# widkyyu/Goal-conditioned-Reinforcement-Learning-with-environmental-and-policy-priors

Measured on AMD Instinct MI355X. Metric: env-steps/sec, higher is better.
Workload: dtype u8

## Files before the change

### goal-conditioned-reinforcement-learning-with-environmental-and-policy-priors_amd/csrc/twoarmy_engine.hip

```cpp

#include <hip/hip_runtime.h>
#include <stdint.h>
#include <stdio.h>
#include <stdlib.h>
#include <string.h>

#include <array>
#include <map>
#include <mutex>
#include <type_traits>
#include <utility>
#include <vector>

#include "launch.h"
#include "philox.h"
#include "twoarmy.h"

namespace {

constexpr int GS = TW_GRID;
constexpr int NC = TW_CELLS;
constexpr int REC = TW_REC_WORDS;

constexpr uint32_t C_EMPTY = 1u;
constexpr uint32_t C_WALL = 2u | (5u << 8);
constexpr uint32_t C_BALL = 6u | (4u << 8);
constexpr uint32_t C_GOAL = 8u | (1u << 8);

constexpr uint32_t M_FREE = 0x3f666666u;
constexpr uint32_t M_WALL = 0xbf666666u;
constexpr uint32_t M_BALL = 0xbf000000u;
constexpr uint32_t M_AGENT = 0x3e99999au;

constexpr int GPW = 33, GPX0 = 8, GPY0 = 16, GPP = 35;
constexpr int GP_WORDS = GPW * GPP;
constexpr int MAT_OFF = 1156;
constexpr int MAT_WORDS = 292;
constexpr int MATC_OFF = MAT_OFF + MAT_WORDS;
constexpr int MATC_BYTES = 304;
constexpr int ENV_WORDS = MATC_OFF + MATC_BYTES / 4;
constexpr int STAGE_WORDS = 220;
constexpr int REC_OBS_OFF = MAT_WORDS * 4;
static_assert(REC_OBS_OFF + 880 == 2048, "matrix row + view-17 image row are exactly 2048 bytes");

enum { R_STEP = 0, R_RISK = 1, R_HIT = 2, R_ROOM2 = 3, R_GOAL = 4 };

struct Params {
    uint8_t *type;
    uint8_t *colour;
    int32_t *rec;
    uint8_t *type_out;
    uint8_t *colour_out;
    int32_t *rec_out;
    int *abnormal;
    int *abnormal_other;
    int only_if_flagged;
    int *fb_count;
    int n_envs;
    int view;
    int variant;
    uint32_t seed_lo, seed_hi;
    uint32_t env_id0;
    int T;
    const int32_t *actions;
    const uint32_t *draws;
    uint8_t *obs;
    float *matrix;
    float *pos;
    float *reward;
    uint8_t *term;
    uint8_t *trunc;
    int obs_pitch;
    int mat_pitch;
    int flags;
    int record;
    const uint32_t *pipe_tab;
};

__device__ __forceinline__ void draw_block(uint32_t k0, uint32_t k1, uint32_t env_id, uint32_t t, uint32_t block,
                                           uint32_t (&w)[4]) {
    w[0] = env_id; w[1] = t; w[2] = block; w[3] = 0x54574F41u;
    philox4x32_10(k0, k1, w[0], w[1], w[2], w[3]);
}

__device__ __forceinline__ uint32_t gen_cell(int x, int y) {
    if (x == 0 || y == 0 || x == GS - 1 || y == GS - 1) return C_WALL;
    if (y == 8) {
        if (x <= 5 || x >= 11) return C_WALL;
        if (x >= 7 && x <= 9) return C_BALL;
        return C_EMPTY;
    }
    if (x == 14 && y == 2) return C_GOAL;
    return C_EMPTY;
}

__device__ __forceinline__ uint32_t mat_of_code(uint32_t code) {
    const uint32_t t = code & 0xffu;
    return t == 2u ? M_WALL : (t == 6u ? M_BALL : M_FREE);
}

struct EnvS {
    int ax, ay, dir, step_count, step_move, m6, m4, pone, patrol, up1, right2, upd_long, upd_horiz, risk,
        first_room2;
    int obx[3], oby[3], o1x[3], o1y[3], o1v, o2x[4], o2y[4], o2v, gx, gy;
    uint32_t t;
    int err, max_steps, episodes, last_reward, last_term, last_trunc;
    int wall_i1, wall_i2;
};

__device__ __forceinline__ void load_env(EnvS &s, const int32_t *r) {
    s.ax = r[TW_AX]; s.ay = r[TW_AY]; s.dir = r[TW_DIR];
    s.step_count = r[TW_STEP_COUNT]; s.step_move = r[TW_STEP_MOVE];
    s.m6 = (int)((uint32_t)s.step_move % 6u); s.m4 = s.step_move & 3;
    s.pone = r[TW_PONE]; s.patrol = r[TW_PATROL]; s.up1 = r[TW_UP1];
    s.right2 = r[TW_RIGHT2]; s.upd_long = r[TW_UPD_LONG]; s.upd_horiz = r[TW_UPD_HORIZ];
    s.risk = r[TW_RISK]; s.first_room2 = r[TW_FIRST_ROOM2];
#pragma unroll
    for (int k = 0; k < 3; ++k) {
        s.obx[k] = r[TW_OBX + k]; s.oby[k] = r[TW_OBY + k];
        s.o1x[k] = r[TW_O1X + k]; s.o1y[k] = r[TW_O1Y + k];
    }
#pragma unroll
    for (int k = 0; k < 4; ++k) { s.o2x[k] = r[TW_O2X + k]; s.o2y[k] = r[TW_O2Y + k]; }
    s.o1v = r[TW_O1_VALID]; s.o2v = r[TW_O2_VALID];
    s.gx = r[TW_GOAL_X]; s.gy = r[TW_GOAL_Y];
    s.t = (uint32_t)r[TW_T]; s.err = r[TW_ERROR]; s.max_steps = r[TW_MAX_STEPS];
    s.episodes = r[TW_EPISODES]; s.last_reward = r[TW_LAST_REWARD];
    s.last_term = r[TW_LAST_TERM]; s.last_trunc = r[TW_LAST_TRUNC];
    s.wall_i1 = r[TW_WALL_I1]; s.wall_i2 = r[TW_WALL_I2];
}

__device__ __forceinline__ void store_env(const EnvS &s, int32_t *r) {
    r[TW_AX] = s.ax; r[TW_AY] = s.ay; r[TW_DIR] = s.dir;
    r[TW_STEP_COUNT] = s.step_count; r[TW_STEP_MOVE] = s.step_move;
    r[TW_PONE] = s.pone; r[TW_PATROL] = s.patrol; r[TW_UP1] = s.up1; r[TW_RIGHT2] = s.right2;
    r[TW_UPD_LONG] = s.upd_long; r[TW_UPD_HORIZ] = s.upd_horiz; r[TW_RISK] = s.risk;
    r[TW_FIRST_ROOM2] = s.first_room2;
#pragma unroll
    for (int k = 0; k < 3; ++k) {
        r[TW_OBX + k] = s.obx[k]; r[TW_OBY + k] = s.oby[k];
        r[TW_O1X + k] = s.o1x[k]; r[TW_O1Y + k] = s.o1y[k];
    }
#pragma unroll
    for (int k = 0; k < 4; ++k) { r[TW_O2X + k] = s.o2x[k]; r[TW_O2Y + k] = s.o2y[k]; }
    r[TW_O1_VALID] = s.o1v; r[TW_O2_VALID] = s.o2v;
    r[TW_GOAL_X] = s.gx; r[TW_GOAL_Y] = s.gy;
    r[TW_T] = (int32_t)s.t; r[TW_ERROR] = s.err; r[TW_MAX_STEPS] = s.max_steps;
    r[TW_EPISODES] = s.episodes; r[TW_LAST_REWARD] = s.last_reward;
    r[TW_LAST_TERM] = s.last_term; r[TW_LAST_TRUNC] = s.last_trunc;
    r[TW_WALL_I1] = s.wall_i1; r[TW_WALL_I2] = s.wall_i2;
}

__device__ __forceinline__ void reset_scalars(EnvS &s) {
#pragma unroll
    for (int k = 0; k < 3; ++k) { s.obx[k] = 7 + k; s.oby[k] = 8; }
    s.o1v = 0; s.o2v = 0;
    s.ax = 3; s.ay = 15; s.dir = 3; s.gx = 14; s.gy = 2;
    s.step_count = 0; s.err = 0;
}

__device__ __forceinline__ bool normal_mode(const EnvS &s) {
    return (s.oby[0] == 8) & (s.oby[1] == 8) & (s.oby[2] == 8) & (s.obx[1] == s.obx[0] + 1) &
           (s.obx[2] == s.obx[0] + 2) & ((unsigned)(s.obx[0] - 2) <= 10u) & (s.dir == 3) &
           ((unsigned)(s.ax - 1) <= 14u) & ((unsigned)(s.ay - 1) <= 14u);
}

__device__ __forceinline__ bool inb(int x, int y) { return (unsigned)x < (unsigned)GS && (unsigned)y < (unsigned)GS; }
__device__ __forceinline__ int gpi(int x, int y) { return (x + GPX0) * GPP + y + GPY0; }

__device__ __forceinline__ void wave_sync() {
    __builtin_amdgcn_fence(__ATOMIC_RELEASE, "wavefront");
    __builtin_amdgcn_wave_barrier();
    __builtin_amdgcn_fence(__ATOMIC_ACQUIRE, "wavefront");
}

__device__ __forceinline__ void store16(void *dst, const uint4 &v) { *reinterpret_cast<uint4 *>(dst) = v; }

__device__ __forceinline__ uint8_t mcode_of(uint32_t mval) {
    return mval == M_WALL ? 1 : (mval == M_BALL ? 2 : (mval == M_AGENT ? 3 : 0));
}
__device__ __forceinline__ uint8_t *mcb(uint32_t *env) { return reinterpret_cast<uint8_t *>(env + MATC_OFF); }
__device__ __forceinline__ const uint8_t *mcb(const uint32_t *env) { return reinterpret_cast<const uint8_t *>(env + MATC_OFF); }

__device__ __forceinline__ void put(uint32_t *env, int x, int y, uint32_t code, uint32_t mval) {
    env[gpi(x, y)] = code;
    env[MAT_OFF + y * GS + x] = mval;
    mcb(env)[y * GS + x] = mcode_of(mval);
}

template <int NB>
__device__ __forceinline__ bool move_group(uint32_t *env, int (&xs)[NB], int (&ys)[NB], int valid, int dx, int dy,
                                           int &err) {
    if (!valid) { err = TW_ENV_TYPE; return false; }
    bool ok = true;
#pragma unroll
    for (int k = 0; k < NB; ++k)
        if (ok) { if (inb(xs[k], ys[k])) put(env, xs[k], ys[k], C_EMPTY, M_FREE); else ok = false; }
    if (!ok) { err = TW_ENV_ASSERT; return false; }
#pragma unroll
    for (int k = 0; k < NB; ++k) {
        const int nx = xs[k] + dx, ny = ys[k] + dy;
        if (inb(nx, ny)) { put(env, nx, ny, C_BALL, M_BALL); xs[k] = nx; ys[k] = ny; }
    }
    return true;
}

__device__ __forceinline__ int advance_counters(EnvS &s) {
    s.t += 1;
    s.step_move += 1;
    s.m6 = s.m6 == 5 ? 0 : s.m6 + 1;
    s.m4 = (s.m4 + 1) & 3;
    return (s.m6 <= 1) ? 1 : (s.m6 <= 3 ? -1 : 0);
}

__device__ __forceinline__ void move_ball_triple(uint32_t *env, EnvS &s, int dxb) {
    uint32_t *row8 = env + gpi(0, 8);
    uint32_t *mrow8 = env + MAT_OFF + 8 * GS;
    uint8_t *crow8 = mcb(env) + 8 * GS;
    const int b0 = s.obx[0], nb = b0 + dxb;
    const int cx = dxb > 0 ? b0 : b0 + 2;
    row8[cx * GPP] = dxb != 0 ? C_EMPTY : C_BALL;
    mrow8[cx] = dxb != 0 ? M_FREE : M_BALL;
    crow8[cx] = dxb != 0 ? 0 : 2;
    row8[nb * GPP] = C_BALL; row8[(nb + 1) * GPP] = C_BALL; row8[(nb + 2) * GPP] = C_BALL;
    mrow8[nb] = M_BALL; mrow8[nb + 1] = M_BALL; mrow8[nb + 2] = M_BALL;
    crow8[nb] = 2; crow8[nb + 1] = 2; crow8[nb + 2] = 2;
    s.obx[0] = nb; s.obx[1] = nb + 1; s.obx[2] = nb + 2;
}

__device__ __forceinline__ bool move_patrols(uint32_t *env, EnvS &s, uint32_t gate, int &err) {
    bool alive = true;
    if (s.upd_long) {
        s.upd_horiz = 0;
        bool go = (s.m4 == 2) || (s.m6 == 3) || (s.m6 == 0);
        if (!go) go = (gate % 10u) == 6u;
        if (go && s.patrol) {
            if (s.up1) {
                alive = move_group<3>(env, s.o1x, s.o1y, s.o1v, 0, -1, err);
                if (alive && s.o1y[0] == 3) s.up1 = 0;
            } else {
                alive = move_group<3>(env, s.o1x, s.o1y, s.o1v, 0, 1, err);
                if (alive && s.o1y[2] == 7) s.up1 = 1;
            }
        }
    }
    if (alive && s.upd_horiz) {
        s.upd_long = 0;
        bool go = (s.m6 != 1);
        if (!go) go = (gate % 10u) == 6u;
        if (go && s.patrol) {
            if (s.right2) {
                alive = move_group<4>(env, s.o2x, s.o2y, s.o2v, 1, 0, err);
                if (alive && s.o2x[3] == 11) s.right2 = 0;
            } else {
                alive = move_group<4>(env, s.o2x, s.o2y, s.o2v, -1, 0, err);
                if (alive && s.o2x[0] == 5) s.right2 = 1;
            }
        }
    }
    return alive;
}

__device__ __forceinline__ float reward_value(int code) {
    return code == R_STEP ? -0.01f : code == R_RISK ? -0.1f : code == R_HIT ? -0.9f : code == R_ROOM2 ? 0.2f : 0.9f;
}

template <typename Fetch>
__device__ __forceinline__ void emit_obs_generic(Fetch fetch, uint32_t *stage, int lane, int V, int ax, int ay,
                                                 int dir, uint8_t *dst) {
    const int VV = V * V, h = V >> 1, nb = VV * 3;
    int topx, topy;
    if (dir == 0) { topx = ax; topy = ay - h; }
    else if (dir == 1) { topx = ax - h; topy = ay; }
    else if (dir == 2) { topx = ax - V + 1; topy = ay - h; }
    else { topx = ax - h; topy = ay - V + 1; }
    const int c_agent = h * V + V - 1;
    const uint32_t off = (uint32_t)(uintptr_t)dst & 3u;
    uint8_t *sb = reinterpret_cast<uint8_t *>(stage) + off;
    for (int c = lane; c < VV; c += 64) {
        const int i = c / V, j = c - i * V;
        int sx, sy;
        if (dir == 0) { sx = V - 1 - j; sy = i; }
        else if (dir == 1) { sx = V - 1 - i; sy = V - 1 - j; }
        else if (dir == 2) { sx = j; sy = V - 1 - i; }
        else { sx = i; sy = j; }
        const int x = topx + sx, y = topy + sy;
        uint32_t v = inb(x, y) ? fetch(x, y) : C_WALL;
        if (c == c_agent) v = C_EMPTY;
        sb[3 * c + 0] = (uint8_t)v;
        sb[3 * c + 1] = (uint8_t)(v >> 8);
        sb[3 * c + 2] = (uint8_t)(v >> 16);
    }
    wave_sync();
    const int first = (4 - (int)off) & 3;
    const int nmid = (nb - first) >> 2;
    const int tail = (nb - first) & 3;
    if (lane < first) dst[lane] = sb[lane];
    {
        uint32_t *gd = reinterpret_cast<uint32_t *>(dst + first);
        const uint32_t *sd = stage + ((off + first) >> 2);
        for (int d = lane; d < nmid; d += 64) gd[d] = sd[d];
    }
    if (lane < tail) dst[first + nmid * 4 + lane] = sb[first + nmid * 4 + lane];
    wave_sync();
}

struct ObsFast {
    int rel4[6];
    uint32_t shift;
    uint32_t andm[4], orm[4];
    int active;
    int chunk;
};

__device__ __forceinline__ ObsFast make_obs_fast(int chunk, int V) {
    ObsFast f;
    const int VV = V * V, h = V >> 1, nb = VV * 3;
    const int nchunks = (nb + 15) >> 4;
    f.active = chunk >= 0 && chunk < nchunks;
    f.chunk = f.active ? chunk : 0;
    const int lane = f.chunk;
    const int s0 = 16 * lane;
    const int c0 = s0 / 3;
    f.shift = 8u * (uint32_t)(s0 - 3 * c0);
    const int c_agent = h * V + V - 1;
#pragma unroll
    for (int k = 0; k < 6; ++k) {
        int c = c0 + k;
// ... 460 lines not shown
    wave_sync();
    if (lane < E) store_env(s, recs + lane * REC);
    wave_sync();
    for (int i = lane; i < E * REC; i += 64) {
        const int e = i / REC;
        if (n0 + e < N) p.rec_out[(size_t)n0 * REC + i] = recs[i];
    }
#pragma unroll
    for (int e = 0; e < E; ++e) {
        if (n0 + e >= N) break;
        const uint32_t *env = lds_env + e * ENV_WORDS;
        const size_t gb = (size_t)(n0 + e) * NC;
        for (int c = lane; c < NC; c += 64) {
            const int y = c / GS, x = c - y * GS;
            const uint32_t v = env[gpi(x, y)];
            p.type_out[gb + c] = (uint8_t)v;
            p.colour_out[gb + c] = (uint8_t)(v >> 8);
        }
    }
}

template <int E, int VARIANT, bool FAST>
__global__ __launch_bounds__(64, (E == 1 ? 4 : 2)) void tw_rollout_kernel(Params p) {
    __shared__ __attribute__((aligned(16))) uint32_t lds_env[E * ENV_WORDS];
    __shared__ __attribute__((aligned(16))) uint32_t stage[STAGE_WORDS];
    __shared__ int32_t recs[E * REC];
    __shared__ int32_t act_lds[64 * E];
    if (p.only_if_flagged) {
        if (*p.abnormal == 0) return;
        if (blockIdx.x == 0 && threadIdx.x == 0) atomicAdd(p.fb_count, 1);
    }
    const int groups = (p.n_envs + E - 1) / E;
    for (int b = blockIdx.x; b < groups; b += gridDim.x) {
        rollout_body<E, VARIANT, FAST>(p, b * E, threadIdx.x, lds_env, stage, recs, act_lds);
        wave_sync();
    }
}


constexpr int PWAVES = 16;
constexpr int PG_MAX = 16;
constexpr int PIPE_WG_TARGET = 256;
constexpr int PCH = 128;
constexpr int PGRP_FLOAT = 1, PGRP_CODE = 4;
constexpr uint32_t REC_VALID = 0x80000000u;

struct Dyn { int b0, pone, i1, i2, patrol, o1y0, o2x0; };
#define LG_RARE(c) __builtin_expect(!!(c), 0)
template <int K>
__device__ __forceinline__ uint32_t lshl_or(uint32_t x, uint32_t acc) {
    uint32_t r;
    asm("v_lshl_or_b32 %0, %1, %2, %3" : "=v"(r) : "v"(x), "n"(K), "v"(acc));
    return r;
}

__device__ __forceinline__ uint32_t static_cell(int x, int y) {
    if (x == 0 || y == 0 || x == GS - 1 || y == GS - 1) return C_WALL;
    if (y == 8) return (x <= 5 || x >= 11) ? C_WALL : C_EMPTY;
    if (x == 14 && y == 2) return C_GOAL;
    return C_EMPTY;
}

__device__ __forceinline__ uint32_t analytic_cell(int x, int y, const Dyn &d) {
    uint32_t c = static_cell(x, y);
    if (y == 8 && (unsigned)(x - d.b0) <= 2u) c = C_BALL;
    if (d.pone && ((((unsigned)(x - 4) <= 1u) & ((unsigned)(y - d.i1) <= 1u)) |
                   (((unsigned)(x - d.i2) <= 1u) & ((unsigned)(y - 11) <= 1u)))) c = C_WALL;
    if (d.patrol && (((x == 12) & ((unsigned)(y - d.o1y0) <= 2u)) |
                     (((unsigned)(x - d.o2x0) <= 1u) & ((unsigned)(y - 4) <= 1u)))) c = C_BALL;
    return c;
}

template <bool V4>
__device__ __forceinline__ bool pipe_state_ok(const EnvS &s) {
    bool ok = normal_mode(s) & ((unsigned)(s.obx[0] - 6) <= 2u) & (s.err == 0) & (s.gx == 14) & (s.gy == 2) &
              (s.max_steps > 0);
    ok &= s.obx[0] == (int)((0x666787u >> (4 * ((uint32_t)s.step_move % 6u))) & 15u);
    if (s.pone) ok &= ((unsigned)(s.wall_i1 - 9) <= 3u) & ((unsigned)(s.wall_i2 - 6) <= 3u);
    if (V4) {
        if (s.patrol) {
            ok &= (s.o1v != 0) & (s.o2v != 0) & (s.o1x[0] == 12) & (s.o1x[1] == 12) & (s.o1x[2] == 12) &
                  (s.o1y[1] == s.o1y[0] + 1) & (s.o1y[2] == s.o1y[0] + 2) & ((unsigned)(s.o1y[0] - 3) <= 2u) &
                  ((unsigned)(s.o2x[0] - 5) <= 5u) & (s.o2x[1] == s.o2x[0] + 1) & (s.o2x[2] == s.o2x[0]) &
                  (s.o2x[3] == s.o2x[0] + 1) & (s.o2y[0] == 4) & (s.o2y[1] == 4) & (s.o2y[2] == 5) & (s.o2y[3] == 5);
        }
    } else {
        ok &= (s.patrol == 0);
    }
    return ok;
}

__device__ __forceinline__ uint32_t pack_record(int ax, int ay, const Dyn &d, int pone_pre, int patrol_pre, int reward,
                                                int terminated, int truncated) {
    return (uint32_t)ax | ((uint32_t)ay << 5) | ((uint32_t)((d.b0 - 6) & 3) << 10) | ((uint32_t)((d.o1y0 - 3) & 3) << 12) |
           ((uint32_t)((d.o2x0 - 5) & 7) << 14) | ((uint32_t)((d.i1 - 9) & 3) << 17) | ((uint32_t)((d.i2 - 6) & 3) << 19) |
           ((uint32_t)pone_pre << 21) | ((uint32_t)d.pone << 22) | ((uint32_t)patrol_pre << 23) |
           ((uint32_t)d.patrol << 24) | ((uint32_t)reward << 25) | ((uint32_t)(terminated != 0) << 28) |
           ((uint32_t)(truncated != 0) << 29);
}

constexpr int PT_IMG = 0, PT_OBS = ENV_WORDS, PT_WORDS = PT_OBS + 2 * 64 * 16;
static_assert(ENV_WORDS % 4 == 0 && ENV_WORDS / 4 <= 6 * 64, "image copied as 6 x dwordx4 per lane");

__global__ __launch_bounds__(64) void tw_pipe_tables_kernel(uint32_t *tab, int V) {
    const int lane = threadIdx.x;
    uint32_t *im = tab + PT_IMG;
    for (int i = lane; i < ENV_WORDS; i += 64) im[i] = 0u;
    __syncthreads();
    for (int i = lane; i < GP_WORDS; i += 64) {
        const int x = i / GPP - GPX0, y = i - (i / GPP) * GPP - GPY0;
        im[i] = inb(x, y) ? static_cell(x, y) : C_WALL;
    }
    for (int c = lane; c < MAT_WORDS; c += 64)
        im[MAT_OFF + c] = c < NC ? mat_of_code(static_cell(c - (c / GS) * GS, c / GS)) : 0u;
    for (int c = lane; c < MATC_BYTES; c += 64)
        mcb(im)[c] = c < NC ? mcode_of(mat_of_code(static_cell(c - (c / GS) * GS, c / GS))) : 0;
    for (int r = 0; r < 2; ++r) {
        const ObsFast f = make_obs_fast(r ? lane - 9 : lane, V);
        uint32_t *o = tab + PT_OBS + (r * 64 + lane) * 16;
        for (int k = 0; k < 6; ++k) o[k] = (uint32_t)f.rel4[k];
        o[6] = f.shift;
        for (int k = 0; k < 4; ++k) { o[7 + k] = f.andm[k]; o[11 + k] = f.orm[k]; }
        o[15] = (uint32_t)f.active;
    }
}

template <int VARIANT, int PG, int LAYOUT>
__global__ __launch_bounds__(64 * PWAVES, 16 / PWAVES) void tw_pipe_kernel(Params p) {
    constexpr bool CODE = LAYOUT == 2;
    constexpr int PGRP = (CODE ? PGRP_CODE : PGRP_FLOAT) < PG ? (CODE ? PGRP_CODE : PGRP_FLOAT) : PG;
    extern __shared__ __attribute__((aligned(16))) uint32_t pipe_lds[];
    uint32_t *img = pipe_lds;
    uint32_t *ring = img + PWAVES * ENV_WORDS;
    int32_t *recs = reinterpret_cast<int32_t *>(ring + PCH * PG);
    volatile int *ctrl = reinterpret_cast<volatile int *>(recs + PG * REC);
    uint32_t *drw = const_cast<uint32_t *>(reinterpret_cast<volatile uint32_t *>(ctrl + 4));

    constexpr bool V4 = VARIANT == 4;
    const int tid = threadIdx.x, lane = tid & 63, wave = tid >> 6;
    const int N = p.n_envs;
    const int n0 = ((gridDim.x & 7) == 0 ? (int)((blockIdx.x & 7) * (gridDim.x >> 3) + (blockIdx.x >> 3)) : (int)blockIdx.x) * PG;
    uint32_t *my_img = img + wave * ENV_WORDS;

    constexpr bool record = LAYOUT == 1;
    const uint4 *tab4 = reinterpret_cast<const uint4 *>(p.pipe_tab);
#pragma unroll
    for (int k = 0; k < 6; ++k)
        if (lane + 64 * k < ENV_WORDS / 4)
            __builtin_amdgcn_global_load_lds(tab4 + lane + 64 * k,
                                             (__attribute__((address_space(3))) void *)(my_img + 256 * k), 16, 0, 0);
    const uint4 *of4 = tab4 + PT_OBS / 4 + ((record ? 64 : 0) + lane) * 4;
    const uint4 ofw0 = of4[0], ofw1 = of4[1], ofw2 = of4[2], ofw3 = of4[3];
    const bool own_env = wave < PG && n0 + wave < N;
    const int ve = min(n0 + (wave < PG ? wave : 0), N - 1);
    const int32_t rec_pre = p.rec[(size_t)ve * REC + (lane < REC ? lane : 0)];
    uint32_t ty_pre[5], co_pre[5];
#pragma unroll
    for (int k = 0; k < 5; ++k) {
        const size_t g = (size_t)ve * NC + min(lane + 64 * k, NC - 1);
        ty_pre[k] = p.type[g]; co_pre[k] = p.colour[g];
    }
    constexpr int NPRE = (PCH * PG + 64 * PWAVES - 1) / (64 * PWAVES);
    int act_pre[NPRE];
    {
        const int len0 = min(PCH, p.T);
#pragma unroll
        for (int k = 0; k < NPRE; ++k) {
            const int i = tid + k * 64 * PWAVES, tl = i / PG, e = i - tl * PG;
            act_pre[k] = p.actions[(size_t)min(tl, len0 - 1) * N + min(n0 + e, N - 1)];
        }
    }
    constexpr bool code_mode = CODE;
    uint8_t *img_bytes = reinterpret_cast<uint8_t *>(my_img);
    if (wave < PG && lane < REC) recs[wave * REC + lane] = own_env ? rec_pre : 0;
    if (tid == 0) { ctrl[0] = 0; ctrl[1] = 0; }
    if (blockIdx.x == 0 && tid == 0) *p.abnormal_other = 0;
    __builtin_amdgcn_s_waitcnt(0x0f70);
    __syncthreads();

    {
        EnvS s;
        load_env(s, recs + (wave < PG ? wave : 0) * REC);
        bool ok = true;
        if (own_env) {
            ok = pipe_state_ok<V4>(s);
            Dyn d = {s.obx[0], s.pone, s.wall_i1, s.wall_i2, s.patrol, s.o1y[0], s.o2x[0]};
#pragma unroll
            for (int k = 0; k < 5; ++k) {
                const int c = lane + 64 * k;
                if (c < NC) ok &= analytic_cell(c - (c / GS) * GS, c / GS, d) == (ty_pre[k] | (co_pre[k] << 8));
            }
        }
        if (__ballot(!ok) != 0ull && lane == 0) atomicOr(p.abnormal, 1);
    }

    ObsFast of;
    of.rel4[0] = (int)ofw0.x; of.rel4[1] = (int)ofw0.y; of.rel4[2] = (int)ofw0.z; of.rel4[3] = (int)ofw0.w;
    of.rel4[4] = (int)ofw1.x; of.rel4[5] = (int)ofw1.y; of.shift = ofw1.z;
    of.andm[0] = ofw1.w; of.andm[1] = ofw2.x; of.andm[2] = ofw2.y; of.andm[3] = ofw2.z;
    of.orm[0] = ofw2.w; of.orm[1] = ofw3.x; of.orm[2] = ofw3.y; of.orm[3] = ofw3.z;
    of.active = (int)ofw3.w; of.chunk = of.active ? (record ? lane - 9 : lane) : 0;
    int dc_xc = 0, dc_yc = 0;
    uint32_t dc_xsh = 0, dc_xmask = 0, dc_ysh = 0, dc_ymask = 0, dc_always = 0, dc_fmask = 0, dc_prebit = 0, dc_postbit = 0;
    uint32_t dc_code = C_BALL, dc_mval = M_BALL;
    const uint8_t dc_mcode = (lane >= 3 && lane < 11) ? 1 : 2;
    if (lane < 3) { dc_always = 1; dc_xc = 6 + lane; dc_xsh = 10; dc_xmask = 3; dc_yc = 8; }
    else if (lane < 7) { const int k = lane - 3; dc_fmask = 1; dc_prebit = 21; dc_postbit = 22; dc_xc = 4 + (k & 1);
                         dc_yc = 9 + (k >> 1); dc_ysh = 17; dc_ymask = 3; dc_code = C_WALL; dc_mval = M_WALL; }
    else if (lane < 11) { const int k = lane - 7; dc_fmask = 1; dc_prebit = 21; dc_postbit = 22; dc_xc = 6 + (k >> 1);
                          dc_xsh = 19; dc_xmask = 3; dc_yc = 11 + (k & 1); dc_code = C_WALL; dc_mval = M_WALL; }
    else if (lane < 14) { dc_fmask = 1; dc_prebit = 23; dc_postbit = 24; dc_xc = 12; dc_yc = 3 + (lane - 11);
                          dc_ysh = 12; dc_ymask = 3; }
    else if (lane < 18) { const int k = lane - 14; dc_fmask = 1; dc_prebit = 23; dc_postbit = 24; dc_xc = 5 + (k & 1);
                          dc_xsh = 14; dc_xmask = 7; dc_yc = 4 + (k >> 1); }
    const int trash_g = (lane % GPW) * GPP + 33 + lane / GPW;
    const int mat_lane_off = (MAT_OFF + 4 * lane) * 4;
    const int mat_laneb_off = (MAT_OFF + 4 * (lane < 9 ? 64 + lane : 72)) * 4;

    const bool lg_active = wave == 0 && lane < PG && n0 + lane < N;
    constexpr uint32_t LG_B0 = 0x019019u;
    constexpr uint32_t LG_GL = 0x3C30F3u;
    constexpr uint32_t LG_GH = 0xFF3FF3u;
    constexpr uint32_t LG_Y1 = 0x64u;
    constexpr uint32_t LG_X2 = 0x0A72C688u;
    constexpr uint32_t GOALW = 14u | (2u << 5);
    struct {
        int step_count, sm_off, risk, max_steps, episodes, last_reward, last_term, last_trunc, i1, i2;
        uint32_t posw, ph2, c1x2, c2x3, pl2, ph3, pm, npone, first_room2, upd_long, upd_horiz, w1, w2, dynw, seenw, t;
    } s;
    bool bad = false;
    {
        const int32_t *r = recs + (lane < PG ? lane : 0) * REC;
        s.posw = (uint32_t)r[TW_AX] | ((uint32_t)r[TW_AY] << 5);
        s.step_count = r[TW_STEP_COUNT]; s.sm_off = r[TW_STEP_MOVE] - s.step_count;
        s.ph2 = 2u * ((uint32_t)r[TW_STEP_MOVE] % 12u);
        s.upd_long = r[TW_UPD_LONG] != 0; s.upd_horiz = r[TW_UPD_HORIZ] != 0;
        s.risk = r[TW_RISK]; s.first_room2 = r[TW_FIRST_ROOM2] != 0; s.max_steps = r[TW_MAX_STEPS];
        s.episodes = r[TW_EPISODES]; s.last_reward = r[TW_LAST_REWARD]; s.last_term = r[TW_LAST_TERM];
        s.last_trunc = r[TW_LAST_TRUNC]; s.t = (uint32_t)r[TW_T];
        const bool pone = r[TW_PONE] != 0;
        s.npone = pone ? 0u : ~0u; s.i1 = r[TW_WALL_I1]; s.i2 = r[TW_WALL_I2];
        const bool patrol = r[TW_PATROL] != 0;
        const int up1 = r[TW_UP1] != 0, right2 = r[TW_RIGHT2] != 0, y1 = r[TW_O1Y], x2 = r[TW_O2X];
        s.w1 = pone ? 0x30u : 0u; s.w2 = pone ? 3u << s.i2 : 0u;
        s.dynw = pone ? (((uint32_t)(s.i1 - 9) & 3u) << 17) | (((uint32_t)(s.i2 - 6) & 3u) << 19) | (1u << 22) : 0u;
        if (patrol) s.dynw |= 1u << 24;
        s.seenw = (s.dynw & ((1u << 22) | (1u << 24))) >> 1;
        s.dynw |= REC_VALID;
        if (V4 && s.upd_long) s.upd_horiz = 0;
        uint32_t c1 = up1 ? 2u : 0u, c2 = right2 ? 0u : 5u;
        if (V4 && patrol) {
            c1 = up1 ? (y1 == 4 ? 3u : 2u) : (y1 == 4 ? 1u : 0u);
            c2 = right2 ? (uint32_t)(x2 - 5) : (uint32_t)(15 - x2);
            bad |= ((unsigned)(y1 - 3) > 2u) | ((unsigned)(x2 - 5) > 5u) | (up1 ? y1 == 3 : y1 == 5) | (right2 ? x2 == 10 : x2 == 5);
            c1 &= 3u; c2 = c2 > 9u ? 0u : c2;
        }
        s.c1x2 = 2u * c1; s.c2x3 = 3u * c2;
        s.pm = (V4 && patrol) ? ~0u : 0u;
        s.pl2 = (V4 && patrol && s.upd_long) ? 2u : 0u; s.ph3 = (V4 && patrol && s.upd_horiz) ? 3u : 0u;
    }
    const bool policy_idx = (p.flags & TW_F_POLICY_IDX) != 0;

    for (int c0 = 0; c0 < p.T; c0 += PCH) {
        const int len = min(PCH, p.T - c0);
#pragma unroll
        for (int k = 0; k < NPRE; ++k) {
            const int i = tid + k * 64 * PWAVES;
            if (i >= len * PG) break;
            const int tl = i / PG, e = i - tl * PG;
            const int act_in = (n0 + e < N) ? (c0 == 0 ? act_pre[k] : p.actions[(size_t)(c0 + tl) * N + n0 + e]) : 0;
            ring[i] = (n0 + e < N) ? 0u : REC_VALID;
            const uint32_t eid = p.env_id0 + (uint32_t)(n0 + e);
            const uint32_t tnow = (uint32_t)recs[e * REC + TW_T] + (uint32_t)(c0 + tl);
            uint32_t w[4], packed = 0;
            if (V4) {
                draw_block(p.seed_lo, p.seed_hi, eid, tnow, 0, w);
                packed = ((w[TW_S_GATE] % 10u) == 6u ? 3u : 0u) | ((w[TW_S_WALL1] & 3u) << 2) | ((w[TW_S_WALL2] & 3u) << 4) |
                         ((w[TW_S_SPAWN] & 3u) << 6);
            }
            draw_block(p.seed_lo, p.seed_hi, eid, tnow, 1, w);
            packed |= ((w[0] & 1u) << 8) | ((w[1] & 1u) << 9);
            int a = act_in;
            const bool neg = a < 0;
            if (policy_idx && a == 4) a = 6;
            if (a >= 7) a = 0;
            const bool raises = neg || ((0x4Fu >> (a & 7)) & 1u) == 0u;
            const int dx = raises ? 0 : (int)((0x1558u >> (2 * a)) & 3u) - 1, dy = raises ? 0 : (int)((0x1585u >> (2 * a)) & 3u) - 1;
            drw[i] = packed | ((raises ? 1u : 0u) << 10) | ((uint32_t)(dx + 32 * dy) << 16);
        }
        __syncthreads();
        if (wave == 0) {
            __builtin_amdgcn_s_setprio(3);
            const uint32_t *drp = drw + (lane < PG ? lane : 0);
            uint32_t *rgp = ring + (lane < PG ? lane : 0);
            uint32_t dr_next = *drp, badw = 0u, last_rec = 0u;
            uint32_t pend = 0u, *pendp = rgp;
            if (lg_active)
#pragma unroll 1
            for (int tl = 0; tl < len; ++tl) {
                const uint32_t dr = dr_next;
                drp += PG;
                dr_next = *drp;
                badw |= dr;
                s.ph2 = s.ph2 == 22u ? 0u : s.ph2 + 2u;
                const uint32_t b0o = (LG_B0 >> s.ph2) & 3u;
                const uint32_t balls = 0x1C0u << b0o;
                if (V4) {
                    s.c1x2 = (s.c1x2 + (((LG_GL >> s.ph2) | dr) & s.pl2)) & 6u;
                    s.c2x3 += ((LG_GH >> s.ph2) | dr) & s.ph3;
                    s.c2x3 = s.c2x3 == 30u ? 0u : s.c2x3;
                }
                uint32_t y1o = (LG_Y1 >> s.c1x2) & 3u, x2o = (LG_X2 >> s.c2x3) & 7u;
                s.step_count += 1;
                const uint32_t tposw = s.posw + (uint32_t)((int32_t)dr >> 16);
                *pendp = pend;
                const int ty = (int)(tposw >> 5);
                uint32_t rb = ty == 8 ? (0x1F83Fu | balls) : 0x10001u;
                rb = (unsigned)(ty - 1) > 14u ? 0x1FFFFu : rb;
                rb |= (unsigned)(ty - s.i1) <= 1u ? s.w1 : 0u;
                rb |= (unsigned)(ty - 11) <= 1u ? s.w2 : 0u;
                if (V4) {
                    rb |= (unsigned)(ty - 3 - (int)y1o) <= 2u ? (s.pm & 0x1000u) : 0u;
                    rb |= (unsigned)(ty - 4) <= 1u ? (s.pm & (0x60u << x2o)) : 0u;
                }
                s.posw = __builtin_amdgcn_ubfe(rb, tposw, 1u) ? s.posw : tposw;
                const uint32_t terminated = tposw == GOALW;
                uint32_t truncated = s.step_count >= s.max_steps;
                const uint32_t seen = s.seenw;
                const int ay = (int)(s.posw >> 5);
                const uint32_t armed = V4 ? (s.npone | ((s.posw - (9u << 5)) & ~s.pm)) : s.npone;
                if (LG_RARE((int32_t)armed < 0)) {
                    if (s.npone && ((s.posw & 31u) > 3u || ay < 14)) {
                        s.i1 = V4 ? 9 + (int)((dr >> 2) & 3u) : 11;
                        s.i2 = V4 ? 6 + (int)((dr >> 4) & 3u) : 8;
                        s.npone = 0u;
                        s.w1 = 0x30u; s.w2 = 3u << s.i2;
                        s.dynw = (s.dynw & ~(15u << 17)) | ((uint32_t)(s.i1 - 9) << 17) | ((uint32_t)(s.i2 - 6) << 19) | (1u << 22);
                        s.seenw |= 1u << 21;
                    }
                    if (V4 && s.pm == 0u && ay <= 8) {
                        const uint32_t dq = (dr >> 6) & 3u;
                        s.c1x2 = 2u + (s.c1x2 & 4u);
                        s.c2x3 = s.c2x3 < 15u ? 3u + 3u * dq : 27u - 3u * dq;
                        y1o = 1u; x2o = 1u + dq;
                        s.pm = ~0u; s.pl2 = s.upd_long ? 2u : 0u; s.ph3 = s.upd_horiz ? 3u : 0u;
                        s.dynw |= 1u << 24;
                        s.seenw |= 1u << 23;
                    }
                }
                uint32_t hitm = ay == 8 ? balls : 0u, riskm = ay == 9 ? balls : 0u;
                if (V4) {
                    const uint32_t colr = (unsigned)(ay - 3 - (int)y1o) <= 2u ? s.pm : 0u, sqr = (unsigned)(ay - 4) <= 1u ? s.pm : 0u;
                    const uint32_t sq = 0x60u << x2o;
                    hitm |= (colr & 0x1000u) | (sqr & sq);
                    riskm |= (colr & 0x800u) | (sqr & ((sq << 1) | (sq >> 1))) | (ay == 6 ? s.pm & sq : 0u);
                }
                const uint32_t hit = __builtin_amdgcn_ubfe(hitm, s.posw, 1u), risky = __builtin_amdgcn_ubfe(riskm, s.posw, 1u);
                uint32_t reward = hit ? (uint32_t)R_HIT : risky;
                truncated |= hit;
                const uint32_t room2 = ay == 7 ? s.first_room2 : 0u;
                reward = room2 ? (uint32_t)R_ROOM2 : reward;
                s.first_room2 &= ~room2;
                const uint32_t isrisk = reward == (uint32_t)R_RISK;
                s.risk += (int)isrisk;
                truncated |= isrisk & (uint32_t)(s.risk > 5);
                const uint32_t rtt = lshl_or<4>(truncated, terminated ? ((uint32_t)R_GOAL | 8u) : reward);
                uint32_t rec = lshl_or<10>(b0o, s.posw | s.dynw | seen);
                if (V4) rec = lshl_or<14>(x2o, lshl_or<12>(y1o, rec));
                rec = lshl_or<25>(rtt, rec);
                if (LG_RARE((terminated | truncated) != 0u)) {
                    const uint32_t ca = (dr >> 8) & 1u, cb = (dr >> 9) & 1u;
                    s.ph2 = 0u; s.sm_off = 0; s.first_room2 = 1u; s.risk = 0;
                    s.c1x2 = 4u - 4u * ca; s.c2x3 = 15u - 15u * ca;
                    s.upd_horiz = 1u - cb; s.upd_long = cb;
                    s.episodes += 1;
                    s.npone = ~0u; s.pm = 0u; s.pl2 = 0u; s.ph3 = 0u; s.w1 = 0u; s.w2 = 0u; s.dynw = REC_VALID; s.seenw = 0u;
                    s.posw = 3u | (15u << 5); s.step_count = 0;
                }
                pend = rec; pendp = rgp;
                rgp += PG;
            }
            if (lg_active) { *pendp = pend; last_rec = pend; }
            if (lg_active) {
                s.t += (uint32_t)len;
                s.last_reward = (int)((last_rec >> 25) & 7u); s.last_term = (int)((last_rec >> 28) & 1u);
                s.last_trunc = (int)((last_rec >> 29) & 1u);
                bad |= ((badw >> 10) & 1u) != 0u;
            }
            if (__ballot(bad) != 0ull && lane == 0) atomicOr(p.abnormal, 1);
            __builtin_amdgcn_s_setprio(0);
        }
        const int ngroups = len * (PG / PGRP);
        while (true) {
            int kg = 0;
            if (lane == 0) kg = atomicAdd(const_cast<int *>(&ctrl[1]), 1);
            kg = __builtin_amdgcn_readfirstlane(kg);
            if (kg >= ngroups) break;
            const int tl = kg / (PG / PGRP), e0 = (kg - tl * (PG / PGRP)) * PGRP;
            const int npoll = e0 == 0 ? PG : PGRP;
            uint32_t rv = REC_VALID;
            while (true) {
                if (lane < npoll) rv = const_cast<volatile uint32_t *>(ring)[tl * PG + e0 + lane];
                if (__ballot((rv & REC_VALID) == 0u) == 0ull) break;
                __builtin_amdgcn_s_sleep(1);
            }
            if (e0 == 0 && lane < PG && n0 + lane < N) {
                const size_t srow = (size_t)(c0 + tl) * N + n0 + lane;
                p.reward[srow] = reward_value((int)((rv >> 25) & 7u));
                p.term[srow] = (uint8_t)((rv >> 28) & 1u);
                p.trunc[srow] = (uint8_t)((rv >> 29) & 1u);
                reinterpret_cast<float2 *>(p.pos)[srow] = make_float2((float)((rv >> 5) & 31u), (float)(rv & 31u));
            }
            const size_t grow = (size_t)(c0 + tl) * N + n0 + e0;
            uint8_t *obs_g = p.obs + grow * (size_t)p.obs_pitch;
            float *mat_g = p.matrix + grow * (size_t)p.mat_pitch;
#pragma unroll 1
            for (int j = 0; j < PGRP; ++j) {
                if (n0 + e0 + j >= N) break;
                const uint32_t r = (uint32_t)__builtin_amdgcn_readlane((int)rv, j);
                const int ax = r & 31, ay = (r >> 5) & 31;
                uint8_t *obs_dst = obs_g + (size_t)j * p.obs_pitch;
                float *mat_dst = mat_g + (size_t)j * p.mat_pitch;
                uint8_t *matc_dst = reinterpret_cast<uint8_t *>(p.matrix) + (grow + j) * (size_t)p.mat_pitch;
                const int x = dc_xc + (int)((r >> dc_xsh) & dc_xmask);
                const int y = dc_yc + (int)((r >> dc_ysh) & dc_ymask);
                const bool pre = (dc_always | ((r >> dc_prebit) & dc_fmask)) != 0u;
                const int gcell = gpi(x, y), mcell = MAT_OFF + y * GS + x;
                const int gidx = pre ? gcell : trash_g, midx = pre ? mcell : trash_g;
                const int ca = MAT_OFF + ay * GS + ax;
                const int bidx = pre ? MATC_OFF * 4 + y * GS + x : trash_g * 4;
                const int bca = lane == 0 ? MATC_OFF * 4 + ay * GS + ax : trash_g * 4;
                my_img[gidx] = dc_code;
                if (code_mode) img_bytes[bidx] = dc_mcode; else my_img[midx] = dc_mval;
                wave_sync();
                if ((((r >> 21) ^ (r >> 22)) & 5u) == 0u) {
                    if (code_mode) img_bytes[bca] = 3;
                    else my_img[lane == 0 ? ca : trash_g] = M_AGENT;
                    wave_sync();
                    const char *base = reinterpret_cast<const char *>(my_img + gpi(ax, ay));
                    uint32_t c[6];
#pragma unroll
                    for (int k = 0; k < 6; ++k) c[k] = *reinterpret_cast<const uint32_t *>(base + of.rel4[k]);
                    uint4 m0 = make_uint4(0u, 0u, 0u, 0u), m1 = m0;
                    if (code_mode) {
                        m0 = *reinterpret_cast<const uint4 *>(img_bytes + MATC_OFF * 4 + 16 * (lane < MATC_BYTES / 16 ? lane : 0));
                    } else {
                        m0 = *reinterpret_cast<const uint4 *>(reinterpret_cast<const char *>(my_img) + mat_lane_off);
                        m1 = *reinterpret_cast<const uint4 *>(reinterpret_cast<const char *>(my_img) + mat_laneb_off);
                    }
                    const uint32_t w0 = c[0] | (c[1] << 24), w1 = (c[1] >> 8) | (c[2] << 16), w2 = (c[2] >> 16) | (c[3] << 8);
                    const uint32_t w3 = c[4] | (c[5] << 24), w4 = c[5] >> 8;
                    uint4 o;
                    o.x = (__builtin_amdgcn_alignbit(w1, w0, of.shift) & of.andm[0]) | of.orm[0];
                    o.y = (__builtin_amdgcn_alignbit(w2, w1, of.shift) & of.andm[1]) | of.orm[1];
                    o.z = (__builtin_amdgcn_alignbit(w3, w2, of.shift) & of.andm[2]) | of.orm[2];
                    o.w = (__builtin_amdgcn_alignbit(w4, w3, of.shift) & of.andm[3]) | of.orm[3];
                    if (record) {
                        uint8_t *rec_dst = reinterpret_cast<uint8_t *>(mat_dst);
                        store16(rec_dst + 16 * lane, m0);
                        uint4 b;
                        b.x = lane < 9 ? m1.x : o.x; b.y = lane < 9 ? m1.y : o.y;
                        b.z = lane < 9 ? m1.z : o.z; b.w = lane < 9 ? m1.w : o.w;
                        if ((lane < 9) | of.active) store16(rec_dst + 1024 + 16 * lane, b);
                    } else if (!code_mode) {
                        if (of.active) store16(obs_dst + 16 * lane, o);
                        store16(mat_dst + 4 * lane, m0);
                        if (lane < 9) store16(mat_dst + 4 * (64 + lane), m1);
                    } else {
                        if (of.active) store16(obs_dst + 16 * lane, o);
                        if (lane < MATC_BYTES / 16) store16(matc_dst + 16 * lane, m0);
                    }
                    wave_sync();
                    my_img[gidx] = C_EMPTY;
                    if (code_mode) img_bytes[bidx] = 0; else my_img[midx] = M_FREE;
                    wave_sync();
                    if (code_mode) img_bytes[bca] = 0;
                    else my_img[lane == 0 ? ca : trash_g] = M_FREE;
                } else {
                    const bool post = (dc_always | ((r >> dc_postbit) & dc_fmask)) != 0u;
                    emit_obs_fast(my_img, ax, ay, of, lane, obs_dst);
                    wave_sync();
                    if (post) { my_img[gcell] = dc_code; my_img[mcell] = dc_mval; mcb(my_img)[y * GS + x] = dc_mcode; }
                    wave_sync();
                    if (code_mode) emit_codes(my_img, ax, ay, lane, matc_dst, true);
                    else emit_matrix_fast(my_img, ax, ay, lane, mat_dst);
                    wave_sync();
                    if (post | pre) { my_img[gcell] = C_EMPTY; my_img[mcell] = M_FREE; mcb(my_img)[y * GS + x] = 0; }
                }
                wave_sync();
            }
        }
        __syncthreads();
        if (tid == 0) { ctrl[0] = 0; ctrl[1] = 0; }
        __syncthreads();
    }

    if (wave == 0 && lane < PG) {
        int32_t *r = recs + lane * REC;
        const int c1 = (int)(s.c1x2 >> 1), c2 = (int)(s.c2x3 / 3u);
        const int up1 = c1 >> 1, right2 = c2 < 5;
        const int patrol = s.pm != 0u, o1y0 = 3 + (int)((LG_Y1 >> s.c1x2) & 3u), o2x0 = 5 + (int)((LG_X2 >> s.c2x3) & 7u);
        r[TW_AX] = (int)(s.posw & 31u); r[TW_AY] = (int)(s.posw >> 5); r[TW_STEP_COUNT] = s.step_count;
        r[TW_STEP_MOVE] = s.step_count + s.sm_off;
        r[TW_UP1] = up1; r[TW_RIGHT2] = right2; r[TW_UPD_LONG] = (int)s.upd_long; r[TW_UPD_HORIZ] = (int)s.upd_horiz;
        r[TW_RISK] = s.risk; r[TW_FIRST_ROOM2] = (int)s.first_room2; r[TW_EPISODES] = s.episodes;
        r[TW_LAST_REWARD] = s.last_reward; r[TW_LAST_TERM] = s.last_term; r[TW_LAST_TRUNC] = s.last_trunc;
        r[TW_T] = (int32_t)s.t; r[TW_ERROR] = 0;
        r[TW_PONE] = s.npone == 0u; r[TW_PATROL] = patrol; r[TW_WALL_I1] = s.i1; r[TW_WALL_I2] = s.i2;
        const int b0_end = 6 + (int)((LG_B0 >> s.ph2) & 3u);
#pragma unroll
        for (int k = 0; k < 3; ++k) { r[TW_OBX + k] = b0_end + k; r[TW_OBY + k] = 8; }
        if (V4) {
            r[TW_O1_VALID] = patrol; r[TW_O2_VALID] = patrol;
            if (patrol) {
#pragma unroll
                for (int k = 0; k < 3; ++k) { r[TW_O1X + k] = 12; r[TW_O1Y + k] = o1y0 + k; }
#pragma unroll
                for (int k = 0; k < 4; ++k) { r[TW_O2X + k] = o2x0 + (k & 1); r[TW_O2Y + k] = 4 + (k >> 1); }
            }
        }
    }
    __syncthreads();
    if (wave < PG && n0 + wave < N) {
        const int32_t *r = recs + wave * REC;
        if (lane < REC) p.rec_out[(size_t)(n0 + wave) * REC + lane] = r[lane];
        Dyn fd = {r[TW_OBX], r[TW_PONE], r[TW_WALL_I1], r[TW_WALL_I2], r[TW_PATROL], r[TW_O1Y], r[TW_O2X]};
        const size_t gb = (size_t)(n0 + wave) * NC;
        for (int c = lane; c < NC; c += 64) {
            const uint32_t v = analytic_cell(c - (c / GS) * GS, c / GS, fd);
            p.type_out[gb + c] = (uint8_t)v;
            p.colour_out[gb + c] = (uint8_t)(v >> 8);
        }
    }
}

__global__ __launch_bounds__(64) void tw_reset_kernel(Params p, const uint8_t *mask, int mode) {
    __shared__ uint32_t cells[NC + 3];
    __shared__ uint32_t stage[STAGE_WORDS];
    const int n = blockIdx.x, lane = threadIdx.x;
    if (mask && !mask[n]) return;
    int32_t *r = p.rec + (size_t)n * REC;
    if (lane == 0) {
        if (mode == 0) {
            for (int k = 0; k < REC; ++k) r[k] = 0;
            r[TW_MAX_STEPS] = 50;
            r[TW_UPD_LONG] = 1; r[TW_RIGHT2] = 1; r[TW_FIRST_ROOM2] = 1;
        }
        for (int k = 0; k < 3; ++k) { r[TW_OBX + k] = 7 + k; r[TW_OBY + k] = 8; }
        r[TW_O1_VALID] = 0; r[TW_O2_VALID] = 0;
        r[TW_AX] = 3; r[TW_AY] = 15; r[TW_DIR] = 3; r[TW_GOAL_X] = 14; r[TW_GOAL_Y] = 2;
        r[TW_STEP_COUNT] = 0; r[TW_ERROR] = 0;
    }
    for (int c = lane; c < NC; c += 64) {
        const int y = c / GS, x = c - y * GS;
        const uint32_t v = gen_cell(x, y);
        cells[c] = v;
        p.type[(size_t)n * NC + c] = (uint8_t)v;
        p.colour[(size_t)n * NC + c] = (uint8_t)(v >> 8);
    }
    wave_sync();
    const uint32_t *cc = cells;
    if (p.obs)
        emit_obs_generic([cc](int x, int y) { return cc[y * GS + x]; }, stage, lane, p.view, 3, 15, 3,
                         p.obs + (size_t)n * p.obs_pitch);
}

__global__ __launch_bounds__(64) void tw_gen_obs_kernel(Params p) {
    __shared__ uint32_t cells[NC + 3];
    __shared__ uint32_t stage[STAGE_WORDS];
    const int n = blockIdx.x, lane = threadIdx.x;
    for (int c = lane; c < NC; c += 64)
        cells[c] = (uint32_t)p.type[(size_t)n * NC + c] | ((uint32_t)p.colour[(size_t)n * NC + c] << 8);
    wave_sync();
    const int32_t *r = p.rec + (size_t)n * REC;
    const int ax = __builtin_amdgcn_readfirstlane(r[TW_AX]), ay = __builtin_amdgcn_readfirstlane(r[TW_AY]);
    const int dir = __builtin_amdgcn_readfirstlane(r[TW_DIR]);
    const uint32_t *cc = cells;
    emit_obs_generic([cc](int x, int y) { return cc[y * GS + x]; }, stage, lane, p.view, ax, ay, dir,
                     p.obs + (size_t)n * p.obs_pitch);
}

__global__ void tw_fill_actions_kernel(Params p, int32_t *out) {
    const int i = blockIdx.x * blockDim.x + threadIdx.x;
    const int total = p.T * p.n_envs;
    if (i >= total) return;
    const int tt = i / p.n_envs, n = i - tt * p.n_envs;
    const uint32_t t = (uint32_t)p.rec[(size_t)n * REC + TW_T] + (uint32_t)tt;
    uint32_t w[4];
    draw_block(p.seed_lo, p.seed_hi, p.env_id0 + (uint32_t)n, t, 2, w);
    out[i] = (int32_t)(w[0] % 5u);
}

}

struct tw_engine {
    int variant, n_envs, view, device;
    uint64_t seed;
    uint32_t env_id0;
    uint8_t *type, *colour;
    int32_t *rec;
    uint8_t *type2, *colour2;
    int32_t *rec2;
    int *abnormal;
    int parity;
    int envs_per_wave;
    int pipeline;
    int *fb_count;
    uint32_t *pipe_tab;
    int last[8];
};

namespace {

struct DeviceGuard {
    int prev = -1;
    bool ok = true;
    explicit DeviceGuard(int dev) {
        if (hipGetDevice(&prev) != hipSuccess) prev = -1;
        if (prev != dev) ok = hipSetDevice(dev) == hipSuccess;
    }
    ~DeviceGuard() { if (prev >= 0) (void)hipSetDevice(prev); }
};

Params base_params(const tw_engine *e) {
    Params p;
    memset(&p, 0, sizeof(p));
    p.type = e->type; p.colour = e->colour; p.rec = e->rec;
    p.type_out = e->type; p.colour_out = e->colour; p.rec_out = e->rec;
    p.abnormal = e->abnormal; p.abnormal_other = e->abnormal + 1; p.only_if_flagged = 0;
    p.fb_count = e->fb_count;
    p.pipe_tab = e->pipe_tab;
    p.n_envs = e->n_envs; p.view = e->view; p.variant = e->variant;
    p.seed_lo = (uint32_t)e->seed; p.seed_hi = (uint32_t)(e->seed >> 32);
    p.env_id0 = e->env_id0;
    p.T = 1;
    p.obs_pitch = e->view * e->view * 3;
    p.mat_pitch = NC;
    return p;
}

bool view_ok(int v) { return v >= 3 && v <= GS && (v & 1); }

int pick_envs_per_wave(const tw_engine *e) {
    if (e->envs_per_wave > 0) return e->envs_per_wave;
    if (e->n_envs >= 2048) return 2;
    return 1;
}

bool params_fast(const tw_engine *e, const Params &p, bool allow_codes) {
    const int chunk = ((e->view * e->view * 3 + 15) >> 4) << 4;
    const bool codes = (p.flags & TW_F_MATRIX_CODE) != 0;
    if (codes && !allow_codes) return false;
    const bool mat_ok = codes ? ((p.mat_pitch & 15) == 0 && p.mat_pitch >= MATC_BYTES)
                              : ((p.mat_pitch & 3) == 0 && p.mat_pitch >= MAT_WORDS);
    return p.obs && p.matrix && p.pos && p.reward && p.term && p.trunc && p.actions && !p.draws &&
           ((uintptr_t)p.obs & 15u) == 0 && (p.obs_pitch & 15) == 0 && p.obs_pitch >= chunk &&
           ((uintptr_t)p.matrix & 15u) == 0 && mat_ok;
}

using KernelFn = void (*)(Params);
constexpr int log2i(int v) { return v > 1 ? 1 + log2i(v >> 1) : 0; }

template <size_t... I>
constexpr std::array<KernelFn, sizeof...(I)> rollout_table(std::index_sequence<I...>) {
    return {{&tw_rollout_kernel<1 << (I / 4), (I / 2) % 2 ? 6 : 4, (I % 2) != 0>...}};
}
constexpr auto ROLLOUT_KERNELS = rollout_table(std::make_index_sequence<12>{});

template <size_t... I>
constexpr std::array<KernelFn, sizeof...(I)> pipe_table(std::index_sequence<I...>) {
    return {{&tw_pipe_kernel<I / 12 ? 6 : 4, 2 << (I % 4), (I / 4) % 3>...}};
}
constexpr auto PIPE_KERNELS = pipe_table(std::make_index_sequence<24>{});

constexpr int PIPE_MIN_T = 8;
constexpr size_t PIPE_LDS_BYTES = (size_t)(PWAVES * ENV_WORDS + PCH * PG_MAX + PG_MAX * REC + 4 + (PCH + 1) * PG_MAX) * 4;

enum { LL_PIPELINED = 0, LL_PG, LL_LAYOUT, LL_PIPE_GRID, LL_E, LL_FAST, LL_SEQ_GRID, LL_T };

int launch_sequential(tw_engine *e, const Params &p, hipStream_t st) {
// ... 380 lines not shown
```

Baseline: 3.003 billion.

## Replace block barriers with lighter LDS barriers and flag-signalled epilogue handoff

Replaces the double __syncthreads plus ctrl reset at the end of each chunk with one raw s_waitcnt+s_barrier, placing the ctrl[1] reset before the mid-chunk barrier. The final chunk's barrier is skipped. Wave 0 now signals completion of the record write-back through an LDS flag instead of a block barrier. The epilogue is also reassigned to a rotated wave (se), so other waves can write their env outputs as soon as the flag is set. This aims to cut barrier overhead per chunk and at kernel exit. The cost is reliance on hand-written memory ordering and spin-waiting, which risks subtle races.

After: 2.994 billion. Within noise of the previous version (-0.3%).

```diff
diff --git a/goal-conditioned-reinforcement-learning-with-environmental-and-policy-priors_amd/csrc/twoarmy_engine.hip b/goal-conditioned-reinforcement-learning-with-environmental-and-policy-priors_amd/csrc/twoarmy_engine.hip
--- a/goal-conditioned-reinforcement-learning-with-environmental-and-policy-priors_amd/csrc/twoarmy_engine.hip
+++ b/goal-conditioned-reinforcement-learning-with-environmental-and-policy-priors_amd/csrc/twoarmy_engine.hip
@@ -174,6 +174,9 @@
     __builtin_amdgcn_fence(__ATOMIC_ACQUIRE, "wavefront");
 }
 
+__device__ __forceinline__ void lds_wait() { asm volatile("s_waitcnt lgkmcnt(0)" ::: "memory"); }
+__device__ __forceinline__ void lds_barrier() { asm volatile("s_waitcnt lgkmcnt(0)\n\ts_barrier" ::: "memory"); }
+
 __device__ __forceinline__ void store16(void *dst, const uint4 &v) { *reinterpret_cast<uint4 *>(dst) = v; }
 
 __device__ __forceinline__ uint8_t mcode_of(uint32_t mval) {
@@ -940,6 +943,8 @@
     const uint4 *of4 = tab4 + PT_OBS / 4 + ((record ? 64 : 0) + lane) * 4;
     const uint4 ofw0 = of4[0], ofw1 = of4[1], ofw2 = of4[2], ofw3 = of4[3];
     const bool own_env = wave < PG && n0 + wave < N;
+    const int se = (wave + PWAVES - 1) & (PWAVES - 1);
+    const bool side_env = se < PG && n0 + se < N;
     const int ve = min(n0 + (wave < PG ? wave : 0), N - 1);
     const int32_t rec_pre = p.rec[(size_t)ve * REC + (lane < REC ? lane : 0)];
     uint32_t ty_pre[5], co_pre[5];
@@ -960,34 +965,6 @@
     }
     constexpr bool code_mode = CODE;
     uint8_t *img_bytes = reinterpret_cast<uint8_t *>(my_img);
-    if (wave < PG && lane < REC) recs[wave * REC + lane] = own_env ? rec_pre : 0;
-    if (tid == 0) { ctrl[0] = 0; ctrl[1] = 0; }
-    if (blockIdx.x == 0 && tid == 0) *p.abnormal_other = 0;
-    __builtin_amdgcn_s_waitcnt(0x0f70);
-    __syncthreads();
-
-    {
-        EnvS s;
-        load_env(s, recs + (wave < PG ? wave : 0) * REC);
-        bool ok = true;
-        if (own_env) {
-            ok = pipe_state_ok<V4>(s);
-            Dyn d = {s.obx[0], s.pone, s.wall_i1, s.wall_i2, s.patrol, s.o1y[0], s.o2x[0]};
-#pragma unroll
-            for (int k = 0; k < 5; ++k) {
-                const int c = lane + 64 * k;
-                if (c < NC) ok &= analytic_cell(c - (c / GS) * GS, c / GS, d) == (ty_pre[k] | (co_pre[k] << 8));
-            }
-        }
-        if (__ballot(!ok) != 0ull && lane == 0) atomicOr(p.abnormal, 1);
-    }
-
-    ObsFast of;
-    of.rel4[0] = (int)ofw0.x; of.rel4[1] = (int)ofw0.y; of.rel4[2] = (int)ofw0.z; of.rel4[3] = (int)ofw0.w;
-    of.rel4[4] = (int)ofw1.x; of.rel4[5] = (int)ofw1.y; of.shift = ofw1.z;
-    of.andm[0] = ofw1.w; of.andm[1] = ofw2.x; of.andm[2] = ofw2.y; of.andm[3] = ofw2.z;
-    of.orm[0] = ofw2.w; of.orm[1] = ofw3.x; of.orm[2] = ofw3.y; of.orm[3] = ofw3.z;
-    of.active = (int)ofw3.w; of.chunk = of.active ? (record ? lane - 9 : lane) : 0;
     int dc_xc = 0, dc_yc = 0;
     uint32_t dc_xsh = 0, dc_xmask = 0, dc_ysh = 0, dc_ymask = 0, dc_always = 0, dc_fmask = 0, dc_prebit = 0, dc_postbit = 0;
     uint32_t dc_code = C_BALL, dc_mval = M_BALL;
@@ -1004,6 +981,35 @@
     const int trash_g = (lane % GPW) * GPP + 33 + lane / GPW;
     const int mat_lane_off = (MAT_OFF + 4 * lane) * 4;
     const int mat_laneb_off = (MAT_OFF + 4 * (lane < 9 ? 64 + lane : 72)) * 4;
+
+    if (wave < PG && lane < REC) recs[wave * REC + lane] = own_env ? rec_pre : 0;
+    if (tid == 0) ctrl[0] = 0;
+    if (blockIdx.x == 0 && tid == 0) *p.abnormal_other = 0;
+    __builtin_amdgcn_s_waitcnt(0x0f70);
+    __syncthreads();
+
+    {
+        EnvS s;
+        load_env(s, recs + (wave < PG ? wave : 0) * REC);
+        bool ok = true;
+        if (own_env) {
+            ok = pipe_state_ok<V4>(s);
+            Dyn d = {s.obx[0], s.pone, s.wall_i1, s.wall_i2, s.patrol, s.o1y[0], s.o2x[0]};
+#pragma unroll
+            for (int k = 0; k < 5; ++k) {
+                const int c = lane + 64 * k;
+                if (c < NC) ok &= analytic_cell(c - (c / GS) * GS, c / GS, d) == (ty_pre[k] | (co_pre[k] << 8));
+            }
+        }
+        if (__ballot(!ok) != 0ull && lane == 0) atomicOr(p.abnormal, 1);
+    }
+
+    ObsFast of;
+    of.rel4[0] = (int)ofw0.x; of.rel4[1] = (int)ofw0.y; of.rel4[2] = (int)ofw0.z; of.rel4[3] = (int)ofw0.w;
+    of.rel4[4] = (int)ofw1.x; of.rel4[5] = (int)ofw1.y; of.shift = ofw1.z;
+    of.andm[0] = ofw1.w; of.andm[1] = ofw2.x; of.andm[2] = ofw2.y; of.andm[3] = ofw2.z;
+    of.orm[0] = ofw2.w; of.orm[1] = ofw3.x; of.orm[2] = ofw3.y; of.orm[3] = ofw3.z;
+    of.active = (int)ofw3.w; of.chunk = of.active ? (record ? lane - 9 : lane) : 0;
 
     const bool lg_active = wave == 0 && lane < PG && n0 + lane < N;
     constexpr uint32_t LG_B0 = 0x019019u;
@@ -1076,7 +1082,9 @@
             const int dx = raises ? 0 : (int)((0x1558u >> (2 * a)) & 3u) - 1, dy = raises ? 0 : (int)((0x1585u >> (2 * a)) & 3u) - 1;
             drw[i] = packed | ((raises ? 1u : 0u) << 10) | ((uint32_t)(dx + 32 * dy) << 16);
         }
-        __syncthreads();
+        if (tid == 0) ctrl[1] = 0;
+        lds_barrier();
+        const bool last_chunk = c0 + PCH >= p.T;
         if (wave == 0) {
             __builtin_amdgcn_s_setprio(3);
             const uint32_t *drp = drw + (lane < PG ? lane : 0);
@@ -1278,42 +1286,45 @@
                 wave_sync();
             }
         }
-        __syncthreads();
-        if (tid == 0) { ctrl[0] = 0; ctrl[1] = 0; }
-        __syncthreads();
-    }
-
-    if (wave == 0 && lane < PG) {
-        int32_t *r = recs + lane * REC;
-        const int c1 = (int)(s.c1x2 >> 1), c2 = (int)(s.c2x3 / 3u);
-        const int up1 = c1 >> 1, right2 = c2 < 5;
-        const int patrol = s.pm != 0u, o1y0 = 3 + (int)((LG_Y1 >> s.c1x2) & 3u), o2x0 = 5 + (int)((LG_X2 >> s.c2x3) & 7u);
-        r[TW_AX] = (int)(s.posw & 31u); r[TW_AY] = (int)(s.posw >> 5); r[TW_STEP_COUNT] = s.step_count;
-        r[TW_STEP_MOVE] = s.step_count + s.sm_off;
-        r[TW_UP1] = up1; r[TW_RIGHT2] = right2; r[TW_UPD_LONG] = (int)s.upd_long; r[TW_UPD_HORIZ] = (int)s.upd_horiz;
-        r[TW_RISK] = s.risk; r[TW_FIRST_ROOM2] = (int)s.first_room2; r[TW_EPISODES] = s.episodes;
-        r[TW_LAST_REWARD] = s.last_reward; r[TW_LAST_TERM] = s.last_term; r[TW_LAST_TRUNC] = s.last_trunc;
-        r[TW_T] = (int32_t)s.t; r[TW_ERROR] = 0;
-        r[TW_PONE] = s.npone == 0u; r[TW_PATROL] = patrol; r[TW_WALL_I1] = s.i1; r[TW_WALL_I2] = s.i2;
-        const int b0_end = 6 + (int)((LG_B0 >> s.ph2) & 3u);
-#pragma unroll
-        for (int k = 0; k < 3; ++k) { r[TW_OBX + k] = b0_end + k; r[TW_OBY + k] = 8; }
-        if (V4) {
-            r[TW_O1_VALID] = patrol; r[TW_O2_VALID] = patrol;
-            if (patrol) {
-#pragma unroll
-                for (int k = 0; k < 3; ++k) { r[TW_O1X + k] = 12; r[TW_O1Y + k] = o1y0 + k; }
-#pragma unroll
-                for (int k = 0; k < 4; ++k) { r[TW_O2X + k] = o2x0 + (k & 1); r[TW_O2Y + k] = 4 + (k >> 1); }
-            }
-        }
-    }
-    __syncthreads();
-    if (wave < PG && n0 + wave < N) {
-        const int32_t *r = recs + wave * REC;
-        if (lane < REC) p.rec_out[(size_t)(n0 + wave) * REC + lane] = r[lane];
-        Dyn fd = {r[TW_OBX], r[TW_PONE], r[TW_WALL_I1], r[TW_WALL_I2], r[TW_PATROL], r[TW_O1Y], r[TW_O2X]};
-        const size_t gb = (size_t)(n0 + wave) * NC;
+        if (!last_chunk) lds_barrier();
+    }
+
+    if (wave == 0) {
+        if (lane < PG) {
+            int32_t *r = recs + lane * REC;
+            const int c1 = (int)(s.c1x2 >> 1), c2 = (int)(s.c2x3 / 3u);
+            const int up1 = c1 >> 1, right2 = c2 < 5;
+            const int patrol = s.pm != 0u, o1y0 = 3 + (int)((LG_Y1 >> s.c1x2) & 3u), o2x0 = 5 + (int)((LG_X2 >> s.c2x3) & 7u);
+            r[TW_AX] = (int)(s.posw & 31u); r[TW_AY] = (int)(s.posw >> 5); r[TW_STEP_COUNT] = s.step_count;
+            r[TW_STEP_MOVE] = s.step_count + s.sm_off;
+            r[TW_UP1] = up1; r[TW_RIGHT2] = right2; r[TW_UPD_LONG] = (int)s.upd_long; r[TW_UPD_HORIZ] = (int)s.upd_horiz;
+            r[TW_RISK] = s.risk; r[TW_FIRST_ROOM2] = (int)s.first_room2; r[TW_EPISODES] = s.episodes;
+            r[TW_LAST_REWARD] = s.last_reward; r[TW_LAST_TERM] = s.last_term; r[TW_LAST_TRUNC] = s.last_trunc;
+            r[TW_T] = (int32_t)s.t; r[TW_ERROR] = 0;
+            r[TW_PONE] = s.npone == 0u; r[TW_PATROL] = patrol; r[TW_WALL_I1] = s.i1; r[TW_WALL_I2] = s.i2;
+            const int b0_end = 6 + (int)((LG_B0 >> s.ph2) & 3u);
+#pragma unroll
+            for (int k = 0; k < 3; ++k) { r[TW_OBX + k] = b0_end + k; r[TW_OBY + k] = 8; }
+            if (V4) {
+                r[TW_O1_VALID] = patrol; r[TW_O2_VALID] = patrol;
+                if (patrol) {
+#pragma unroll
+                    for (int k = 0; k < 3; ++k) { r[TW_O1X + k] = 12; r[TW_O1Y + k] = o1y0 + k; }
+#pragma unroll
+                    for (int k = 0; k < 4; ++k) { r[TW_O2X + k] = o2x0 + (k & 1); r[TW_O2Y + k] = 4 + (k >> 1); }
+                }
+            }
+        }
+        lds_wait();
+        if (lane == 0) ctrl[0] = 1;
+    }
+    if (side_env) {
+        while (ctrl[0] == 0) __builtin_amdgcn_s_sleep(2);
+        wave_sync();
+        const int32_t *r = recs + se * REC;
+        if (lane < REC) p.rec_out[(size_t)(n0 + se) * REC + lane] = r[lane];
+        const Dyn fd = {r[TW_OBX], r[TW_PONE], r[TW_WALL_I1], r[TW_WALL_I2], r[TW_PATROL], r[TW_O1Y], r[TW_O2X]};
+        const size_t gb = (size_t)(n0 + se) * NC;
         for (int c = lane; c < NC; c += 64) {
             const uint32_t v = analytic_cell(c - (c / GS) * GS, c / GS, fd);
             p.type_out[gb + c] = (uint8_t)v;
```
